# lhotse-speech/lhotse

Hardware: AMD Instinct MI355X
Metric: cuts/sec (10 s @16 kHz -> 80-dim log-mel fbank) (higher is better)
Workload: dtype f32

## Files before the change

### lhotse_amd/csrc/hipfeat.hip

```cpp
#include "../../include/hipfeat.h"

#include <hip/hip_runtime.h>

#include <algorithm>
#include <atomic>
#include <cmath>
#include <cstdarg>
#include <cstdio>
#include <cstring>
#include <map>
#include <mutex>
#include <new>
#include <string>
#include <vector>

#include "common.hpp"
#include "kernel_generic.hpp"
#include "fft512_common.hpp"
#include "kernel_fft512b.hpp"
#include "kernel_fft512c.hpp"
#include "kernel_fft1024c.hpp"
#include "kernel_fft2048c.hpp"
#include "plan_tables.hpp"
#include "kernel_resample.hpp"
#include "resample_tables.hpp"
#include "kernel_minibatch.hpp"
#include "kernel_mix.hpp"
#include "kernel_reverb.hpp"
#include "kernel_specaug.hpp"
#include "kernel_whisper2.hpp"
#include "kernel_whisper3.hpp"
#include "kernel_fft256.hpp"
#include "kernel_fft256c.hpp"
#include "kernel_wave.hpp"
#include "host_bulk.hpp"

using namespace hipfeat;

static thread_local char g_err[512] = "";

static inline const char* route_env(const char* name) { return getenv(name); }
#ifdef HIPFEAT_EXPERIMENTS
static inline const char* exp_env(const char* name) { return getenv(name); }
#else
static inline const char* exp_env(const char*) { return nullptr; }
#endif

static hipfeat_status fail(hipfeat_status st, const char* fmt, ...) {
  va_list ap;
  va_start(ap, fmt);
  vsnprintf(g_err, sizeof(g_err), fmt, ap);
  va_end(ap);
  return st;
}

#define HIP_TRY(expr)                                                                          \
  do {                                                                                         \
    hipError_t e_ = (expr);                                                                    \
    if (e_ != hipSuccess)                                                                      \
      return fail(HIPFEAT_ERR_HIP, "%s failed: %s (%s:%d)", #expr, hipGetErrorName(e_), __FILE__, __LINE__); \
  } while (0)

struct DeviceGuard {
  int prev = -1;
  bool ok = true;
  explicit DeviceGuard(int dev) {
    if (hipGetDevice(&prev) != hipSuccess) prev = -1;
    if (prev != dev) ok = (hipSetDevice(dev) == hipSuccess);
  }
  ~DeviceGuard() {
    int cur = -1;
    if (prev >= 0 && hipGetDevice(&cur) == hipSuccess && cur != prev) (void)hipSetDevice(prev);
  }
};

struct StagingSlot {
  void* h = nullptr;
  void* d = nullptr;
  size_t cap = 0;
  hipEvent_t ev = nullptr;
  bool busy = false;
};

enum class Route {
  Generic,
  Fft512b,
  Fft256b,
  Wave,
  Whisper2,
  Fft512c,
  Fft1024c,
  Whisper3,
  Fft2048c,
  Fft256c,
};

struct hipfeat_plan {
  hipfeat_config cfg{};
  int device = 0;
  int feature_dim = 0;
  int K = 0, H = 0, log2H = 0;
  bool pow2 = false;
  int npad_left = 0;
  std::string kernel_name = "generic";
  int blocks_per_cu = 0;
  Route route = Route::Generic;
  const void* fn = nullptr;
  const void* fn_flat = nullptr;
  int block = 0;
  size_t lds = 0;
  float* d_window = nullptr;
  float2* d_tw = nullptr;
  float* d_mel = nullptr;
  int2* d_mel_range = nullptr;
  float* d_dct = nullptr;
  float* d_lifter = nullptr;
  int fpb = 8;
  int span = 0, off_z = 0, off_p = 0, off_tw = 0, off_stat = 0, off_mel = 0;
  float* d_mel_a4 = nullptr;
  float* d_dct_consts = nullptr;
  int lm_stride = 0, dct_groups = 0, dct_floats = 0;
  int tiles_per_block = 4;
  int xs_floats = 0;
  int const_floats = 0;
  float* d_lds_consts = nullptr;
  float* d_mel_a = nullptr;
  WaveWork* d_work = nullptr;
  float* d_c_shared = nullptr;
  int c_shared_floats = 0, c_wtab_off = 0, c_ltab_off = 0, c_xs_floats = 0;
  int fpb_unit = 0, c_rounds_max = 0;
  int w_nsets = 0, w_steps[kWMaxSets] = {}, w_step0[kWMaxSets] = {};
  float* d_x_twp = nullptr;
  int x_waves = 0, x_tws_off = 0, x_tw32_off = 0;
  float* d_mel_t = nullptr;
  int wave_blob_floats = 0;
  bool wave_dct_in_lds = false;
  float* d_wh2_cs = nullptr;
  float* d_wh2_tw = nullptr;
  float* d_wh2_mel = nullptr;
  int32_t* d_wh2_sched = nullptr;
  mutable std::mutex mu;
  mutable StagingSlot slots[4];
  mutable int next_slot = 0;
  mutable float* d_scratch_wave = nullptr;
  mutable size_t scratch_wave_cap = 0;
  mutable float* d_scratch_out = nullptr;
  mutable size_t scratch_out_cap = 0;
};

struct hipfeat_layout {
  int device = 0;
  int64_t batch = 0;
  int64_t total_frames = 0;
  int64_t total_blocks = 0;
  int64_t out_row_stride = 0;
  int uniform_bpc = 0;
  int fpb = 0, fpb_unit = 0;
  CutDesc* d_cuts = nullptr;
  bool owns = true;
  std::vector<int64_t> num_frames;
  std::vector<int32_t> block_cut;
  bool flat = false;
  int64_t total_quads = 0;
  unsigned char* d_norm = nullptr;
  int norm_slots = 0;
  mutable std::atomic<unsigned> norm_next{0};
};
constexpr int kNormSlots = 4;
static size_t norm_slot_bytes(const hipfeat_layout* lay) { return (2 * (size_t)lay->total_blocks + (size_t)lay->batch) * 4; }

extern "C" HIPFEAT_API int32_t hipfeat_abi_version(void) { return HIPFEAT_ABI_VERSION; }
extern "C" HIPFEAT_API const char* hipfeat_last_error(void) { return g_err; }

extern "C" HIPFEAT_API hipfeat_status hipfeat_device_count(int32_t* count) {
  if (!count) return fail(HIPFEAT_ERR_INVALID, "count is NULL");
  int n = 0;
  hipError_t e = hipGetDeviceCount(&n);
  if (e != hipSuccess) {
    *count = 0;
    return fail(HIPFEAT_ERR_HIP, "hipGetDeviceCount failed: %s", hipGetErrorName(e));
  }
  *count = n;
  return HIPFEAT_OK;
}

extern "C" HIPFEAT_API int64_t hipfeat_num_frames(int64_t num_samples, int32_t frame_length, int32_t frame_shift,
                                      int32_t snip_edges) {
  if (frame_shift <= 0 || frame_length <= 0 || num_samples < 0) return 0;
  if (snip_edges) return num_samples < frame_length ? 0 : 1 + (num_samples - frame_length) / frame_shift;
  return (num_samples + frame_shift / 2) / frame_shift;
}

extern "C" HIPFEAT_API hipfeat_status hipfeat_check_length(int64_t padded_len, int32_t frame_length, int32_t frame_shift,
                                               int32_t snip_edges) {
  if (snip_edges) return HIPFEAT_OK;
  const int64_t t = hipfeat_num_frames(padded_len, frame_length, frame_shift, 0);
  if (t <= 0)
    return fail(HIPFEAT_ERR_TOO_SHORT, "waveform of %lld samples yields no frames", (long long)padded_len);
  const int64_t npad_left = (frame_length - frame_shift) / 2;
  const int64_t npad_right = (t - 1) * frame_shift + frame_length - padded_len - npad_left;
  if (npad_left > padded_len || npad_right > padded_len)
    return fail(HIPFEAT_ERR_TOO_SHORT,
                "waveform of %lld samples is shorter than the reflect padding (%lld left, %lld right)",
                (long long)padded_len, (long long)npad_left, (long long)npad_right);
  return HIPFEAT_OK;
}

// ... 100 lines not shown
  std::copy(t.w_step0, t.w_step0 + 4, p->w_step0);
  p->fpb_unit = t.waves * frames;
  p->fpb = p->fpb_unit * rounds;
  p->c_rounds_max = rounds_max;
  if ((st = claim(p, route, fn, 64 * t.waves, t.lds)) != HIPFEAT_OK) return st;
  p->kernel_name = head + strf(" lds=%zuB blocks/CU=%d mel4=%dx%d", t.lds, p->blocks_per_cu, t.sch_nsets, t.sch_steps);
  return HIPFEAT_OK;
}

static hipfeat_status claim_tile(hipfeat_plan* p, Route route, const void* fn, const TileTables& t, int tile_frames, const char* kernel) {
  const hipfeat_config& c = p->cfg;
  const bool mfcc = c.kind == HIPFEAT_MFCC, spec = c.kind == HIPFEAT_SPECTROGRAM || c.kind == HIPFEAT_LOG_SPECTROGRAM;
  hipfeat_status st;
  if ((st = upload(&p->d_lds_consts, t.consts.data(), t.consts.size())) != HIPFEAT_OK) return st;
  if (route == Route::Fft512b && (st = upload(&p->d_mel_a, t.mel_a.data(), t.mel_a.size())) != HIPFEAT_OK) return st;
  if ((st = upload(&p->d_work, t.work, 4)) != HIPFEAT_OK) return st;
  if ((st = upload(&p->d_mel_a4, t.mel_a4.data(), t.mel_a4.size())) != HIPFEAT_OK) return st;
  if (mfcc && (st = upload(&p->d_dct_consts, t.dct.data(), t.dct.size())) != HIPFEAT_OK) return st;
  p->tiles_per_block = 16;
  p->fpb = tile_frames * p->tiles_per_block;
  p->const_floats = (int)t.consts.size();
  p->xs_floats = t.xs_floats;
  p->lm_stride = t.lm_stride;
  p->dct_groups = t.dct_groups;
  p->dct_floats = (int)t.dct.size();
  if ((st = claim(p, route, fn, 256, t.lds)) != HIPFEAT_OK) return st;
  p->kernel_name = strf("%s<%d,%d> %s lds=%zuB blocks/CU=%d", kernel, t.nrows, mfcc ? 1 : (spec ? 2 : 0), mfcc ? "mfcc" : (spec ? "spectrogram" : "fbank"), t.lds,
                        p->blocks_per_cu);
  return HIPFEAT_OK;
}

static bool fft512c_has_flat(int nrows, int N) { return nrows == 13 && N >= 384; }

template <int MODE>
static const void* fft512c_pick(int nrows, int N, bool flat) {
  if (flat && fft512c_has_flat(nrows, N)) return entry<fft512c_kernel<13, 12, MODE, true>>();
  if (nrows == 10) return entry<fft512c_kernel<10, 0, MODE>>();
  if (nrows == 13 && N >= 384) return entry<fft512c_kernel<13, 12, MODE>>();
  if (nrows == 13) return entry<fft512c_kernel<13, 0, MODE>>();
  return entry<fft512c_kernel<16, 0, MODE>>();
}
static const void* fft512c_dispatch(int mode, int nrows, int N, bool flat) {
  return mode == 0 ? fft512c_pick<0>(nrows, N, flat)
                   : (mode == 1 ? fft512c_pick<1>(nrows, N, flat) : (mode == 2 ? fft512c_pick<2>(nrows, N, flat) : fft512c_pick<3>(nrows, N, flat)));
}

static hipfeat_status setup_fft512c(hipfeat_plan* p, const PlanInputs& in, int nrows) {
  const bool mfcc = p->cfg.kind == HIPFEAT_MFCC;
  if (mfcc && (in.M > 4 * kCDctChunks || in.C > 64 || !in.dct)) return HIPFEAT_OK;
  const WaveAutoTables t = build_fft512c_tables(in, nrows, {kCPRowStride, kCMaxSets, kCMaxSteps, kCWaves, kCRegion}, kCDctChunks, kCDctChunksSmall);
  if (!t.fits || t.lds > 80 * 1024 || (t.xs_floats >> 8) > 6) return HIPFEAT_OK;
  hipfeat_status st = claim_wave_auto(p, Route::Fft512c, fft512c_dispatch(t.mode, nrows, in.N, false), t, 4, 8, 16,
                                      strf("fft512c_kernel<%d> %s", nrows, mfcc ? "mfcc" : "fbank"));
  if (st == HIPFEAT_OK && fft512c_has_flat(nrows, in.N)) {
    p->fn_flat = fft512c_dispatch(t.mode, nrows, in.N, true);
    hipError_t e = ensure_dynamic_lds(p->fn_flat, t.lds);
    if (e != hipSuccess) return fail(HIPFEAT_ERR_HIP, "hipFuncSetAttribute(dynamic LDS = %zu B) failed: %s", t.lds, hipGetErrorName(e));
  }
  return st;
}

static hipfeat_status setup_fft512(hipfeat_plan* p, const PlanInputs& in) {
  const hipfeat_config& c = p->cfg;
  const char* force = route_env("HIPFEAT_FORCE_GENERIC");
  if (force && force[0] == '1') return HIPFEAT_OK;
  const bool mfcc = c.kind == HIPFEAT_MFCC;
  const bool spec = c.kind == HIPFEAT_SPECTROGRAM || c.kind == HIPFEAT_LOG_SPECTROGRAM;
  if (c.kind > HIPFEAT_MFCC || c.fft_length != 512 || (in.shift & 1) || in.N < 32 || c.use_energy || (!spec && c.use_fft_mag))
    return HIPFEAT_OK;
  if (mfcc && (in.M > 8 * kMaxDctGroups || in.C > 64)) return HIPFEAT_OK;
  const int need = (in.N + 31) / 32;
  const int nrows = need <= 10 ? 10 : (need <= 13 ? 13 : 16);
  if ((in.M + 15) / 16 > 8) return HIPFEAT_OK;

  if (!spec) {
    const char* var = route_env("HIPFEAT_FFT512_VARIANT");
    if (!(var && var[0] == 'b')) {
      hipfeat_status stc = setup_fft512c(p, in, nrows);
      if (stc != HIPFEAT_OK || p->route == Route::Fft512c) return stc;
    }
  }
  const TileTables t = build_tile_tables(in, nrows, {16, kPRowStride, kMaxGroups0, kMaxGroups1, kTileFrames, kBWaveRegion, false});
  if (!t.fits || t.lds > 160 * 1024) return HIPFEAT_OK;
  const void* fn;
  if (mfcc)
    fn = nrows == 10 ? entry<fft512b_kernel<10, 1>>() : (nrows == 13 ? entry<fft512b_kernel<13, 1>>() : entry<fft512b_kernel<16, 1>>());
  else if (spec)
    fn = nrows == 10 ? entry<fft512b_kernel<10, 2>>() : (nrows == 13 ? entry<fft512b_kernel<13, 2>>() : entry<fft512b_kernel<16, 2>>());
  else
    fn = nrows == 10 ? entry<fft512b_kernel<10, 0>>() : (nrows == 13 ? entry<fft512b_kernel<13, 0>>() : entry<fft512b_kernel<16, 0>>());
  return claim_tile(p, Route::Fft512b, fn, t, kTileFrames, "fft512b_kernel");
}

static hipfeat_status setup_fft1024c(hipfeat_plan* p, const PlanInputs& in) {
  const hipfeat_config& c = p->cfg;
  const int N = in.N, shift = in.shift;
  const bool librosa = c.kind == HIPFEAT_LIBROSA_FBANK;
  if ((c.kind != HIPFEAT_FBANK && !librosa) || c.fft_length != 1024 || (shift & 1) || N < 32 * 17 || c.use_energy ||
      (c.use_fft_mag && !librosa) || route_env("HIPFEAT_FORCE_GENERIC") || route_env("HIPFEAT_NO_WAVE_AUTONOMOUS"))
    return HIPFEAT_OK;
  const int need = (N + 31) / 32;
  const int nrows = need <= 20 ? 20 : (need <= 26 ? 26 : 32);
  static const int kFixedSteps[5][3] = {{0, 0, 0}, {24, 16, 8}, {24, 16, 8}, {24, 24, 8}, {16, 16, 8}};
  int want = 0;
  if (route_env("HIPFEAT_NO_FIXED_SCHEDULE")) want = 0;
  else if (nrows == 32) want = !c.remove_dc_offset && c.preemph_coeff == 0.0f ? 4 : 0;
// ... 337 lines not shown
  lay->flat = ragged && !no_flat && plan->fn_flat;
  lay->total_quads = 0;
  lay->block_cut.clear();
  if (lay->flat) {
    int64_t quads = 0;
    for (int64_t b = 0; b < batch; ++b) {
      if (quads > INT32_MAX - (1 << 24)) return fail(HIPFEAT_ERR_INVALID, "batch too large for one launch");
      descs[(size_t)b].first_block = (int32_t)quads;
      quads += (lay->num_frames[(size_t)b] + 3) / 4;
    }
    static const int forced = exp_env("HIPFEAT_ROUNDS") ? atoi(exp_env("HIPFEAT_ROUNDS")) : 0;
    const int64_t slots = 256LL * std::max(plan->blocks_per_cu, 1);
    const int waves_per_wg = plan->fpb_unit / 4;
    int rounds = plan->c_rounds_max;
    if (forced >= 1 && forced <= plan->c_rounds_max) {
      rounds = forced;
    } else {
      double best = -1.0;
      for (int r = std::min(2, plan->c_rounds_max); r <= plan->c_rounds_max; ++r) {
        const int64_t nb = (quads + (int64_t)waves_per_wg * r - 1) / ((int64_t)waves_per_wg * r);
        const double waves = nb >= 8 * slots ? (double)nb / (double)slots : (double)((nb + slots - 1) / slots);
        const double cost = waves * (0.64 + r);
        if (best < 0.0 || cost <= best * (1.0 + 1e-9)) {
          best = cost;
          rounds = r;
        }
      }
    }
    fpb = plan->fpb_unit * rounds;
    const int64_t qpw = (int64_t)waves_per_wg * rounds;
    blocks = (quads + qpw - 1) / qpw;
    lay->total_quads = quads;
    lay->block_cut.resize((size_t)blocks);
    int64_t cutp = 0;
    for (int64_t g = 0; g < blocks; ++g) {
      const int64_t q = g * qpw;
      while (cutp + 1 < batch && descs[(size_t)cutp + 1].first_block <= q) ++cutp;
      lay->block_cut[(size_t)g] = (int32_t)cutp;
    }
    uniform = 0;
  } else {
    for (int64_t b = 0; b < batch; ++b) {
      if (blocks > INT32_MAX - (1 << 24)) return fail(HIPFEAT_ERR_INVALID, "batch too large for one launch");
      descs[(size_t)b].first_block = (int32_t)blocks;
      const int64_t nb = (lay->num_frames[(size_t)b] + fpb - 1) / fpb;
      blocks += nb;
      if (uniform == -1) uniform = (int)nb;
      else if (uniform != (int)nb) uniform = 0;
    }
  }
  lay->batch = batch;
  lay->total_frames = row;
  lay->total_blocks = blocks;
  lay->out_row_stride = out_row_stride;
  lay->uniform_bpc = uniform > 0 ? uniform : -1;
  if (uniform <= 0 && !lay->flat) {
    lay->block_cut.resize((size_t)blocks);
    for (int64_t b = 0; b < batch; ++b) {
      const int64_t b0 = descs[(size_t)b].first_block, b1 = b + 1 < batch ? descs[(size_t)b + 1].first_block : blocks;
      std::fill(lay->block_cut.begin() + b0, lay->block_cut.begin() + b1, (int32_t)b);
    }
  }
  lay->fpb = fpb;
  lay->fpb_unit = plan->fpb_unit;
  lay->device = plan->device;
  return HIPFEAT_OK;
}

extern "C" HIPFEAT_API hipfeat_status hipfeat_layout_create(const hipfeat_plan* plan, int64_t batch, const int64_t* h_wave_offsets,
                                                const int64_t* h_num_samples, const int64_t* h_padded_len,
                                                const int64_t* h_out_rows, int64_t out_row_stride, void* stream,
                                                hipfeat_layout** layout) {
  if (!layout) return fail(HIPFEAT_ERR_INVALID, "layout pointer is NULL");
  *layout = nullptr;
  hipfeat_layout* lay = new (std::nothrow) hipfeat_layout();
  if (!lay) return fail(HIPFEAT_ERR_INVALID, "out of host memory");
  std::vector<CutDesc> descs;
  hipfeat_status st = build_descs(plan, batch, h_wave_offsets, h_num_samples, h_padded_len, h_out_rows, out_row_stride, descs, lay);
  if (st != HIPFEAT_OK) {
    delete lay;
    return st;
  }
  DeviceGuard g(plan->device);
  const size_t map_bytes = (lay->block_cut.size() * sizeof(int32_t) + 15) & ~(size_t)15;
  const size_t desc_bytes = std::max<size_t>(descs.size(), 1) * sizeof(CutDesc) + map_bytes;
  const size_t norm_bytes = plan->route == Route::Whisper3 ? (size_t)kNormSlots * norm_slot_bytes(lay) : 0;
  std::vector<unsigned char> blob(desc_bytes + norm_bytes, 0);
  if (!descs.empty()) std::memcpy(blob.data(), descs.data(), descs.size() * sizeof(CutDesc));
  if (map_bytes) std::memcpy(blob.data() + descs.size() * sizeof(CutDesc), lay->block_cut.data(), lay->block_cut.size() * sizeof(int32_t));
  hipError_t e = hipMalloc(reinterpret_cast<void**>(&lay->d_cuts), blob.size());
  if (e == hipSuccess && !descs.empty()) {
    e = hipMemcpyAsync(lay->d_cuts, blob.data(), blob.size(), hipMemcpyHostToDevice, (hipStream_t)stream);
    if (e == hipSuccess) e = hipStreamSynchronize((hipStream_t)stream);
  }
  if (norm_bytes) {
    lay->d_norm = reinterpret_cast<unsigned char*>(lay->d_cuts) + desc_bytes;
    lay->norm_slots = kNormSlots;
  }
  if (e != hipSuccess) {
    (void)hipFree(lay->d_cuts);
    delete lay;
    return fail(HIPFEAT_ERR_HIP, "layout upload failed: %s", hipGetErrorName(e));
  }
  *layout = lay;
  return HIPFEAT_OK;
}
// ... 113 lines not shown
      wp.dct = plan->d_dct;
      wp.lifter = plan->d_lifter;
      wp.out_stride = lay->out_row_stride;
      wp.num_cuts = (int32_t)lay->batch;
      wp.uniform_bpc = lay->uniform_bpc;
      wp.frames_per_wave = plan->fpb / 4;
      wp.N = c.frame_length;
      wp.shift = c.frame_shift;
      wp.H = plan->H;
      wp.K = plan->K;
      wp.M = c.num_filters;
      wp.C = c.num_ceps;
      wp.kind = librosa ? (int)HIPFEAT_FBANK : c.kind;
      wp.flags = (c.remove_dc_offset ? F_REMOVE_DC : 0) | (c.use_energy ? F_USE_ENERGY : 0) | (c.raw_energy ? F_RAW_ENERGY : 0) |
                 (c.use_fft_mag ? F_FFT_MAG : 0) | (c.apply_lifter ? F_LIFTER : 0) | (librosa ? (F_CENTER | F_LOG10) : 0);
      wp.npad_left = plan->npad_left;
      wp.preemph = c.preemph_coeff;
      wp.log_energy_floor = c.energy_floor > 0.0f ? logf(c.energy_floor) : -INFINITY;
      wp.mel_floor = c.mel_floor;
      wp.log_offset = c.log_offset;
      arg = &wp;
      break;
    case Route::Whisper2:
      w2.wave = d_wave;
      w2.out = d_out;
      w2.cuts = lay->d_cuts;
      w2.window = plan->d_window;
      w2.cs = plan->d_wh2_cs;
      w2.tw = plan->d_wh2_tw;
      w2.mel_a = plan->d_wh2_mel;
      w2.out_stride = lay->out_row_stride;
      w2.num_cuts = (int32_t)lay->batch;
      w2.uniform_bpc = lay->uniform_bpc;
      w2.M = c.num_filters;
      w2.mel_floor = c.mel_floor;
      w2.sched = plan->d_wh2_sched;
      arg = &w2;
      break;
    case Route::Whisper3:
      fill_wave_autonomous(w3, plan, lay, d_wave, d_out);
      w3.cs = plan->d_wh2_cs;
      w3.total_blocks = (int32_t)lay->total_blocks;
      if (lay->d_norm) {
        unsigned char* slot = lay->d_norm + (size_t)(lay->norm_next.fetch_add(1u) % (unsigned)lay->norm_slots) * norm_slot_bytes(lay);
        w3.wg_stat = reinterpret_cast<float*>(slot);
        w3.cut_done = reinterpret_cast<uint32_t*>(slot + 2 * (size_t)lay->total_blocks * sizeof(float));
      }
      arg = &w3;
      break;
    case Route::Fft512c:
      cp.dct_tab = plan->d_dct_consts;
      cp.C = c.num_ceps;
      cp.total_quads = (int32_t)lay->total_quads;
      [[fallthrough]];
    case Route::Fft256c:
      fill_wave_autonomous(cp, plan, lay, d_wave, d_out);
      fill_frames(cp, plan);
      arg = &cp;
      break;
    case Route::Fft1024c:
      fill_wave_autonomous(kp, plan, lay, d_wave, d_out);
      fill_frames(kp, plan);
      kp.nsets = plan->w_nsets;
      for (int s2 = 0; s2 < kWMaxSets; ++s2) kp.steps[s2] = plan->w_steps[s2], kp.step0[s2] = plan->w_step0[s2];
      arg = &kp;
      break;
    case Route::Fft2048c:
      fill_wave_autonomous(xp, plan, lay, d_wave, d_out);
      fill_frames(xp, plan);
      xp.twp = plan->d_x_twp;
      xp.waves = plan->x_waves;
      xp.tws_off = plan->x_tws_off;
      xp.tw32_off = plan->x_tw32_off;
      xp.nsets = plan->w_nsets;
      for (int s2 = 0; s2 < kXMaxSets; ++s2) xp.steps[s2] = plan->w_steps[s2], xp.step0[s2] = plan->w_step0[s2];
      arg = &xp;
      break;
    case Route::Fft512b:
    case Route::Fft256b:
      bp.wave = d_wave;
      bp.out = d_out;
      bp.cuts = lay->d_cuts;
      bp.lds_consts = plan->d_lds_consts;
      bp.mel_a = plan->d_mel_a4;
      bp.work = plan->d_work;
      bp.out_stride = lay->out_row_stride;
      bp.num_cuts = (int32_t)lay->batch;
      bp.uniform_bpc = lay->uniform_bpc;
      bp.tiles_per_block = plan->tiles_per_block;
      bp.N = c.frame_length;
      bp.shift = c.frame_shift;
      bp.npad_left = plan->npad_left;
      bp.M = c.num_filters;
      bp.flags = (c.remove_dc_offset ? F_REMOVE_DC : 0) | (c.use_fft_mag ? F_FFT_MAG : 0) | (c.kind == HIPFEAT_LOG_SPECTROGRAM ? F_LOG_SPEC : 0);
      bp.log_offset = c.log_offset;
      bp.preemph = c.preemph_coeff;
      bp.mel_floor = c.mel_floor;
      bp.xs_floats = plan->xs_floats;
      bp.const_floats = plan->const_floats;
      bp.dct_consts = plan->d_dct_consts;
      bp.C = c.num_ceps;
      bp.lm_stride = plan->lm_stride;
      bp.dct_groups = plan->dct_groups;
      bp.dct_floats = plan->dct_floats;
      arg = &bp;
      break;
  }
  const void* fn = lay->flat && plan->fn_flat ? plan->fn_flat : plan->fn;
  void* args[] = {arg};
  DeviceGuard g(plan->device);
  set_lds_poison(plan->lds);
  (void)hipLaunchKernel(fn, dim3((unsigned)lay->total_blocks), dim3(plan->block), args, plan->lds, stream);
  HIP_TRY(hipGetLastError());
  if (whisper && !(plan->route == Route::Whisper3 && lay->d_norm)) {
    hipLaunchKernelGGL(whisper_norm_kernel, dim3((unsigned)lay->batch), dim3(1024), 0, stream, lay->d_cuts, d_out, lay->out_row_stride,
                       (int32_t)c.num_filters, (int32_t)c.frame_shift);
    HIP_TRY(hipGetLastError());
  }
  return HIPFEAT_OK;
}

extern "C" HIPFEAT_API hipfeat_status hipfeat_extract_layout(const hipfeat_plan* plan, const hipfeat_layout* layout,
                                                 const float* d_wave, float* d_out, void* stream) {
  if (!plan || !layout) return fail(HIPFEAT_ERR_INVALID, "plan/layout is NULL");
  return launch(plan, layout, d_wave, d_out, (hipStream_t)stream);
}

__global__ __launch_bounds__(256) void fill_padding_kernel(const CutDesc* __restrict__ cuts, float* __restrict__ out, int64_t row_stride,
                                                           int32_t rows_per_cut, int32_t feature_dim, float value) {
  const CutDesc cd = cuts[blockIdx.y];
  const int64_t n = (int64_t)(rows_per_cut - cd.num_frames) * feature_dim;
  float* __restrict__ base = out + (cd.out_row + cd.num_frames) * row_stride;
  for (int64_t i = (int64_t)blockIdx.x * 256 + threadIdx.x; i < n; i += (int64_t)gridDim.x * 256) {
    const int64_t r = i / feature_dim;
    base[r * row_stride + (i - r * feature_dim)] = value;
  }
}

__global__ __launch_bounds__(256) void pcm16_to_float_kernel(const int16_t* __restrict__ in, float* __restrict__ out, int64_t n) {
  const int64_t n8 = n >> 3;
  const bool aligned = ((reinterpret_cast<uintptr_t>(in) & 15) == 0) && ((reinterpret_cast<uintptr_t>(out) & 15) == 0);
  constexpr float k = 1.0f / 32768.0f;
  if (aligned) {
    for (int64_t i = (int64_t)blockIdx.x * 256 + threadIdx.x; i < n8; i += (int64_t)gridDim.x * 256) {
      const int4 v = reinterpret_cast<const int4*>(in)[i];
      const int w[4] = {v.x, v.y, v.z, v.w};
      float4 a, b;
      a.x = (float)(int16_t)(w[0] & 0xffff) * k; a.y = (float)(w[0] >> 16) * k;
      a.z = (float)(int16_t)(w[1] & 0xffff) * k; a.w = (float)(w[1] >> 16) * k;
      b.x = (float)(int16_t)(w[2] & 0xffff) * k; b.y = (float)(w[2] >> 16) * k;
      b.z = (float)(int16_t)(w[3] & 0xffff) * k; b.w = (float)(w[3] >> 16) * k;
      reinterpret_cast<float4*>(out)[2 * i] = a;
      reinterpret_cast<float4*>(out)[2 * i + 1] = b;
    }
    for (int64_t i = (n8 << 3) + (int64_t)blockIdx.x * 256 + threadIdx.x; i < n; i += (int64_t)gridDim.x * 256) out[i] = (float)in[i] * k;
  } else {
    for (int64_t i = (int64_t)blockIdx.x * 256 + threadIdx.x; i < n; i += (int64_t)gridDim.x * 256) out[i] = (float)in[i] * k;
  }
}

extern "C" HIPFEAT_API hipfeat_status hipfeat_pcm16_to_float(const int16_t* d_pcm, float* d_wave, int64_t num_samples, void* stream) {
  if (num_samples < 0 || (num_samples > 0 && (!d_pcm || !d_wave))) return fail(HIPFEAT_ERR_INVALID, "bad pcm16 arguments");
  if (num_samples == 0) return HIPFEAT_OK;
  const int64_t blocks = std::min<int64_t>((num_samples / 8 + 255) / 256 + 1, 256 * 32);
  hipLaunchKernelGGL(pcm16_to_float_kernel, dim3((unsigned)blocks), dim3(256), 0, (hipStream_t)stream, d_pcm, d_wave, num_samples);
// ... 1306 lines not shown
```

### lhotse_amd/csrc/kernel_fft512c.hpp

```cpp
#pragma once
#include "common.hpp"
#include "fft_common.hpp"

namespace hipfeat {

constexpr int kCExRowStride = 34;
constexpr int kCExFrameStride = 8 * kCExRowStride + 16;
constexpr int kCPRowStride = 272;
constexpr int kCRegion = 4 * kCExFrameStride + 16;
constexpr int kCMaxSets = 2;
constexpr int kCMaxSteps = 16;
constexpr int kCWaves = 8;
constexpr int kCLmStride = 48;
constexpr int kCDctChunks = 10;
constexpr int kCDctChunksSmall = 6;

struct Fft512cParams {
  const float* wave;
  float* out;
  const CutDesc* cuts;
  const float* shared_consts;
  int64_t out_stride;
  int32_t num_cuts, uniform_bpc;
  int32_t frames_per_block, rounds;
  int32_t N, shift, npad_left, M, flags;
  float preemph, mel_floor;
  int32_t shared_floats;
  int32_t wtab_off, ltab_off;
  int32_t xs_floats;
  const float* dct_tab;
  int32_t C;
  int32_t total_quads;
};

#ifdef HIPFEAT_PHASE_TIMERS
#define HFC_T(i) { const unsigned long long tt_ = __builtin_readcyclecounter(); hfc_acc[i] += tt_ - hfc_last; hfc_last = tt_; }
#else
#define HFC_T(i)
#endif
#define HFC_SEP() asm volatile("")
__device__ __forceinline__ int mul24(int a, int b) { return (int)__umul24((unsigned)a, (unsigned)b); }

template <int NROWS, int NFULL, int MODE, bool FLAT = false>
__global__ __launch_bounds__(64 * kCWaves, 4) void fft512c_kernel(const Fft512cParams p) {
  extern __shared__ __attribute__((aligned(16))) float smem[];
  HF_POISON_LDS(smem);
  const v2* cwin = reinterpret_cast<const v2*>(smem);
  const v2* ctwp = cwin + NROWS * 16;
  const v2* ctws = ctwp + 256;
  const float* wtab = smem + p.wtab_off;
  const float* ltab = smem + p.ltab_off;

  const int tid = threadIdx.x;
  const int lane = tid & 63;
  const int wv = __builtin_amdgcn_readfirstlane(tid >> 6);

  const int blk = blockIdx.x;
  int cut, fb;
  if (FLAT) {
    cut = __builtin_amdgcn_readfirstlane(block_cut_map(p.cuts, p.num_cuts)[blk]);
    fb = 0;
  } else if (p.uniform_bpc > 0) {
    cut = blk / p.uniform_bpc;
    fb = blk - cut * p.uniform_bpc;
  } else {
    cut = p.uniform_bpc < 0 ? block_cut_map(p.cuts, p.num_cuts)[blk] : find_cut(p.cuts, p.num_cuts, blk);
    fb = blk - p.cuts[cut].first_block;
  }
  CutDesc cd = FLAT ? load_cut_uniform(p.cuts + cut) : p.cuts[cut];
  const int N = p.N, shift = p.shift;

  for (int i = tid; i < p.shared_floats; i += 64 * kCWaves) smem[i] = p.shared_consts[i];
  float* xs = smem + p.shared_floats + wv * (p.xs_floats + kCRegion);
  float* myreg = xs + p.xs_floats;
  const bool dc = (p.flags & F_REMOVE_DC) != 0;
  const float inv_n = 1.0f / (float)N;
  const float c = p.preemph;

  auto stage_span = [&](const CutDesc& cd, int f0, unsigned lane4) {
    const float* __restrict__ w = p.wave + cd.wave_off;
    const int64_t j0 = (int64_t)f0 * shift - p.npad_left;
    if (j0 >= 0 && j0 + p.xs_floats <= cd.num_samples) {
      const char* src = reinterpret_cast<const char*>(w + j0);
      const int nfull = p.xs_floats >> 8;
#pragma unroll
      for (int ch = 0; ch < 6; ++ch) {
        if (ch < nfull)
          __builtin_amdgcn_global_load_lds((const __attribute__((address_space(1))) void*)(src + ((unsigned)ch * 1024u + 4u * lane4)),
                                           (__attribute__((address_space(3))) void*)(xs + ch * 256), 16, 0, 0);
      }
      if ((unsigned)nfull * 256u + lane4 < (unsigned)p.xs_floats)
        __builtin_amdgcn_global_load_lds((const __attribute__((address_space(1))) void*)(src + ((unsigned)nfull * 1024u + 4u * lane4)),
                                         (__attribute__((address_space(3))) void*)(xs + nfull * 256), 16, 0, 0);
    } else {
      for (int i = (int)(lane4 >> 2); i < p.xs_floats; i += 64) xs[i] = load_sample(w, j0 + i, cd.num_samples, cd.padded_len);
    }
  };

  const int first_frame = fb * p.frames_per_block + 4 * wv;
  int quad = 0, next_first = 0, f0_flat = 0;
  int cut_n = 0, quad_n = 0, next_first_n = 0, f0_n = 0;
  CutDesc cd_n = cd;
  auto advance = [&](int q, int& c, CutDesc& d, int& nfirst) {
    while (c + 1 < p.num_cuts && q >= nfirst) {
      ++c;
      d = load_cut_uniform(p.cuts + c);
      nfirst = c + 1 < p.num_cuts ? __builtin_amdgcn_readfirstlane(p.cuts[c + 1].first_block) : p.total_quads;
    }
  };
  if (FLAT) {
    quad = blk * (p.frames_per_block >> 2) + wv;
    next_first = cut + 1 < p.num_cuts ? __builtin_amdgcn_readfirstlane(p.cuts[cut + 1].first_block) : p.total_quads;
    advance(quad, cut, cd, next_first);
    f0_flat = 4 * (quad - cd.first_block);
    cut_n = cut, cd_n = cd, next_first_n = next_first, quad_n = quad + kCWaves;
    advance(quad_n, cut_n, cd_n, next_first_n);
    f0_n = 4 * (quad_n - cd_n.first_block);
  }
  __syncthreads();
  if (FLAT ? quad < p.total_quads : first_frame < cd.num_frames) stage_span(cd, FLAT ? f0_flat : first_frame, (unsigned)lane * 4u);

  constexpr bool kMfcc = MODE == 2 || MODE == 3;
  constexpr int DCH = MODE == 3 ? kCDctChunksSmall : kCDctChunks;
#ifdef HIPFEAT_ABL_MFCC_TWS
  constexpr bool kTwsExp = MODE == 2 && NROWS <= 13;
#else
  constexpr bool kTwsExp = false;
#endif
  constexpr int DREG = kTwsExp ? 6 : (MODE == 2 && NROWS > 13) ? 5 : DCH;
  constexpr bool kDctLate = DREG < DCH;
  constexpr bool kRegTw = !kMfcc && NROWS <= 13;
  constexpr bool kRegTws = kRegTw || (MODE == 3 && NROWS <= 13) || kTwsExp;
  v2 twpreg[kRegTw ? 16 : 1], twsreg[kRegTws ? 8 : 1];
  if (kRegTw) {
#pragma unroll
    for (int k1 = 1; k1 < 16; ++k1) twpreg[k1] = ctwp[k1 * 16 + (lane & 15)];
  }
  if (kRegTws) {
#pragma unroll
    for (int k2 = 0; k2 < 8; ++k2) twsreg[k2] = ctws[k2 * 16 + (lane & 15)];
  }
  f32x4 dw[kMfcc ? DREG : 1];
  float lift = 1.0f;
  if (kMfcc) {
#pragma unroll
    for (int c4 = 0; c4 < DREG; ++c4) dw[c4] = *reinterpret_cast<const f32x4*>(p.dct_tab + (c4 * 64 + lane) * 4);
    lift = p.dct_tab[DCH * 256 + lane];
  }
#ifdef HIPFEAT_PHASE_TIMERS
  unsigned long long hfc_acc[8] = {0, 0, 0, 0, 0, 0, 0, 0}, hfc_last = __builtin_readcyclecounter();
#endif
  for (int r = 0; r < p.rounds; ++r) {
    const int f0 = FLAT ? f0_flat : first_frame + 4 * kCWaves * r;
    if (FLAT ? quad >= p.total_quads : f0 >= cd.num_frames) break;
    const int nf = min(4, cd.num_frames - f0);

    if (r == 0)
    __builtin_amdgcn_s_waitcnt(0x0F70);
    HFC_T(0);
    int lane_o = lane;
    asm volatile("" : "+v"(lane_o));
    const int q = lane_o & 15, g = lane_o >> 4;

    int early_poff[2] = {0, 0};
    v2 Z[16];
    {
      const float* x = xs + mul24(g, shift) + 2 * q;
      v2 z[16];
      v2 win[NROWS];
      v2 sum2 = {0.f, 0.f};
#pragma unroll
      for (int n1 = 0; n1 < NROWS; ++n1) {
        z[n1] = *reinterpret_cast<const v2*>(x + 32 * n1);
        HFC_SEP();
      }
#pragma unroll
      for (int n1 = 0; n1 < NROWS; ++n1) {
        win[n1] = cwin[n1 * 16 + q];
        HFC_SEP();
      }
      float pv[NROWS];
#pragma unroll
      for (int n1 = 0; n1 < NROWS; ++n1) pv[n1] = n1 == 0 ? x[q == 0 ? 0 : -1] : x[32 * n1 - 1];
      asm volatile("s_waitcnt lgkmcnt(0)" ::: "memory");
      HFC_T(1);
      if (FLAT) {
        if (r + 1 < p.rounds && quad_n < p.total_quads) stage_span(cd_n, f0_n, (unsigned)lane_o * 4u);
      } else if (r + 1 < p.rounds && f0 + 4 * kCWaves < cd.num_frames) {
        stage_span(cd, f0 + 4 * kCWaves, (unsigned)lane_o * 4u);
      }

#pragma unroll
      for (int n1 = NFULL; n1 < NROWS; ++n1) {
        if (32 * (n1 + 1) > N) {
          const int m0 = 32 * n1 + 2 * q;
          if (m0 >= N) z[n1].x = 0.f;
          if (m0 + 1 >= N) z[n1].y = 0.f;
        }
      }
      {
        v2 sa = z[0], sb = z[1], sc = z[2], sd = z[3];
#pragma unroll
        for (int n1 = 4; n1 < NROWS; ++n1) {
          if ((n1 & 3) == 0) sa += z[n1];
          if ((n1 & 3) == 1) sb += z[n1];
          if ((n1 & 3) == 2) sc += z[n1];
          if ((n1 & 3) == 3) sd += z[n1];
        }
        sum2 = (sa + sb) + (sc + sd);
      }
      float mu = 0.f;
      if (dc) mu = row16_sum(sum2.x + sum2.y) * inv_n;
      {
        const float nc = -c, mu1 = (1.0f - c) * mu;
#pragma unroll
        for (int n1 = 0; n1 < NROWS; ++n1) {
          v2 t;
          asm("v_fma_f32 %0, %1, %2, %3" : "=v"(t.x) : "s"(nc), "v"(pv[n1]), "v"(z[n1].x));
          asm("v_fma_f32 %0, %1, %2, %3" : "=v"(t.y) : "s"(nc), "v"(z[n1].x), "v"(z[n1].y));
          z[n1] = (t - v2{mu1, mu1}) * win[n1];
        }
      }
#pragma unroll
      for (int n1 = NROWS; n1 < 16; ++n1) z[n1] = v2{0.f, 0.f};
      v2 a[16];
      fft16(z, a);
#pragma unroll
      for (int h = 0; h < 2; ++h) {
        v2 tw[8];
        if (kRegTw) {
#pragma unroll
          for (int rr = 0; rr < 8; ++rr) tw[rr] = twpreg[8 * h + rr];
        } else {
#pragma unroll
          for (int rr = 0; rr < 8; ++rr) {
            tw[rr] = ctwp[(8 * h + rr) * 16 + q];
            HFC_SEP();
          }
        }
#pragma unroll
        for (int rr = (h == 0 ? 1 : 0); rr < 8; ++rr) a[8 * h + rr] = cmul2(a[8 * h + rr], tw[rr]);
      }

// ... 141 lines not shown
      if (MODE != 0) acc[0] += acc[1];
      float val[S][4];
#pragma unroll
      for (int s = 0; s < S; ++s) {
        mel4_reduce_floor(acc[s], lt_m4[s], lt_m8[s], p.mel_floor, val[s]);
#pragma unroll
        for (int i = 0; i < 4; ++i) val[s][i] = fast_log(val[s][i]);
      }
#pragma unroll
      for (int s = 0; s < S; ++s) {
        const int col = lt_col[s];
        if (kMfcc) {
#pragma unroll
          for (int i = 0; i < 4; ++i) lm[i] = val[s][i];
        } else if (col < p.M) {
          mel4_store_saddr<4>(orow, (unsigned)col, p.out_stride, nf, val[s]);
        }
      }
    }
    if (kMfcc) {
      float* lmrow = myreg;
      const int col = lt_col[0];
      if (col < p.M) {
#pragma unroll
        for (int i = 0; i < 4; ++i) lmrow[i * kCLmStride + col] = lm[i];
      }
      __builtin_amdgcn_fence(__ATOMIC_RELEASE, "wavefront");
      __builtin_amdgcn_wave_barrier();
      __builtin_amdgcn_fence(__ATOMIC_ACQUIRE, "wavefront");
      f32x4 al[DCH];
#pragma unroll
      for (int c4 = 0; c4 < DCH; ++c4) al[c4] = *reinterpret_cast<const f32x4*>(lmrow + (lane_o & 3) * kCLmStride + 4 * c4);
      f32x4 d0 = {0.f, 0.f, 0.f, 0.f}, d1 = {0.f, 0.f, 0.f, 0.f};
#pragma unroll
      for (int c4 = 0; c4 < DCH; ++c4) {
#pragma unroll
        for (int i = 0; i < 4; i += 2) {
          const f32x4 w4 = (kDctLate && c4 >= DREG) ? dwx[c4 >= DREG ? c4 - DREG : 0] : dw[c4 < DREG ? c4 : 0];
          d0 = __builtin_amdgcn_mfma_f32_4x4x1f32(al[c4][i], w4[i], d0, 0, 0, 0);
          d1 = __builtin_amdgcn_mfma_f32_4x4x1f32(al[c4][i + 1], w4[i + 1], d1, 0, 0, 0);
        }
      }
      d0 += d1;
      if (lane_o < p.C) {
#pragma unroll
        for (int i = 0; i < 4; ++i)
          if (i < nf) orow[i * p.out_stride + lane_o] = d0[i] * lift;
      }
    }
    HFC_T(6);
#ifdef HIPFEAT_PHASE_TIMERS
    hfc_acc[7] += 1;
#endif
    if (FLAT) {
      quad = quad_n, cut = cut_n, cd = cd_n, next_first = next_first_n, f0_flat = f0_n;
      quad_n += kCWaves;
      advance(quad_n, cut_n, cd_n, next_first_n);
      f0_n = 4 * (quad_n - cd_n.first_block);
    }
  }
#ifdef HIPFEAT_PHASE_TIMERS
  if (lane == 0 && g_phase_buf) {
    unsigned long long* o = g_phase_buf + ((size_t)blockIdx.x * kCWaves + wv) * 8;
    for (int i = 0; i < 8; ++i) o[i] = hfc_acc[i];
  }
#endif
}

}
```

Measured before the change: 2.961 million.

## Make fft512c workgroups persistent over multiple blocks with a cost-model grid size

Adds a host cost model that picks how many logical blocks each workgroup processes, shrinking the launch grid. The fft512c kernel now walks blocks in a grid-stride loop and keeps the double-buffered staging of the next span running across block boundaries. The goal is to amortise per-workgroup startup (constant loading into LDS, initial staging) and to soften the tail effect. The risk is worse load balance when the model picks K>1, plus extra position-tracking state that adds registers.

```diff
diff --git a/lhotse_amd/csrc/blocks_per_wg.hpp b/lhotse_amd/csrc/blocks_per_wg.hpp
--- /dev/null
+++ b/lhotse_amd/csrc/blocks_per_wg.hpp
@@ -0,0 +1,122 @@
+#pragma once
+#include <algorithm>
+#include <cstdint>
+#include <vector>
+
+#if defined(__HIPCC__)
+#define HFB_HD __host__ __device__ inline __attribute__((always_inline))
+#else
+#define HFB_HD inline
+#endif
+
+namespace hipfeat {
+
+constexpr double kWgStartupRounds = 0.64;
+constexpr double kMeasuredStartupRounds = 0.0;
+constexpr double kStaticStrideTail = 0.09;
+
+struct BpwTerms { double startup, tail; };
+constexpr BpwTerms kBpwAsSetUp{kWgStartupRounds, 0.0}, kBpwMeasured{kMeasuredStartupRounds, kStaticStrideTail};
+
+inline int64_t bpw_grid(int64_t total_blocks, int64_t K) { return (total_blocks + std::max<int64_t>(K, 1) - 1) / std::max<int64_t>(K, 1); }
+
+inline double bpw_cost(int64_t grid, int64_t K, int64_t slots, int rounds, BpwTerms t) {
+  const double waves = K == 1 && grid >= 8 * slots ? (double)grid / (double)slots : (double)((grid + slots - 1) / slots);
+  return waves * (t.startup + (double)K * rounds) + (K > 1 ? t.tail * (double)K * rounds : 0.0);
+}
+
+inline int64_t choose_blocks_per_wg(int64_t total_blocks, int64_t slots, int rounds, BpwTerms t = kBpwMeasured) {
+  slots = std::max<int64_t>(slots, 1);
+  if (total_blocks <= slots) return 1;
+  int64_t best_k = 1;
+  double best = bpw_cost(total_blocks, 1, slots, rounds, t);
+  const int64_t wmax = std::min<int64_t>((total_blocks + slots - 1) / slots, 64);
+  for (int64_t w = wmax; w >= 1; --w) {
+    const int64_t K = (total_blocks + w * slots - 1) / (w * slots);
+    const double cost = bpw_cost(bpw_grid(total_blocks, K), K, slots, rounds, t);
+    if (cost < best * (1.0 - 1e-9) || (cost <= best * (1.0 + 1e-9) && K > best_k)) best = cost, best_k = K;
+  }
+  return best_k;
+}
+
+inline int64_t layout_blocks_per_wg(int64_t total_blocks, int64_t slots, int rounds, int64_t forced) {
+  if (total_blocks <= 0) return 1;
+  if (forced > 0) return std::min(forced, total_blocks);
+  return choose_blocks_per_wg(total_blocks, slots, rounds);
+}
+
+HFB_HD uint32_t walk_block(uint32_t g, uint32_t j, uint32_t grid) { return g + j * grid; }
+HFB_HD int percut_first_frame(int fb, int frames_per_block, int wv, int r, int waves) { return fb * frames_per_block + 4 * (wv + waves * r); }
+HFB_HD int flat_quad(int blk, int frames_per_block, int wv, int r, int waves) { return blk * (frames_per_block >> 2) + wv + waves * r; }
+
+struct WalkLayout {
+  std::vector<int64_t> num_frames;
+  std::vector<int64_t> first_block;
+  std::vector<int32_t> block_cut;
+  bool flat = false;
+  int rounds = 0, waves = 8;
+  int64_t total_blocks = 0, total_quads = 0;
+  int frames_per_block() const { return 4 * waves * rounds; }
+};
+
+inline WalkLayout walk_layout(const int64_t* num_frames, int64_t batch, int rounds, int waves, bool flat) {
+  WalkLayout l;
+  l.flat = flat, l.rounds = rounds, l.waves = waves;
+  l.num_frames.assign(num_frames, num_frames + batch);
+  l.first_block.resize((size_t)batch);
+  const int64_t fpb = l.frames_per_block(), qpw = fpb / 4;
+  if (flat) {
+    for (int64_t b = 0; b < batch; ++b) l.first_block[(size_t)b] = l.total_quads, l.total_quads += (num_frames[b] + 3) / 4;
+    l.total_blocks = (l.total_quads + qpw - 1) / qpw;
+    int64_t cutp = 0;
+    for (int64_t g = 0; g < l.total_blocks; ++g) {
+      while (cutp + 1 < batch && l.first_block[(size_t)cutp + 1] <= g * qpw) ++cutp;
+      l.block_cut.push_back((int32_t)cutp);
+    }
+  } else {
+    for (int64_t b = 0; b < batch; ++b) {
+      l.first_block[(size_t)b] = l.total_blocks;
+      const int64_t nb = (num_frames[b] + fpb - 1) / fpb;
+      l.total_blocks += nb;
+      l.block_cut.insert(l.block_cut.end(), (size_t)nb, (int32_t)b);
+    }
+  }
+  return l;
+}
+
+inline bool walk_locate(const WalkLayout& l, int64_t blk, int wv, int r, int64_t* cut, int64_t* first_frame) {
+  if (blk < 0 || blk >= l.total_blocks) return false;
+  int64_t c = l.block_cut[(size_t)blk];
+  if (l.flat) {
+    const int64_t quad = flat_quad((int)blk, l.frames_per_block(), wv, r, l.waves);
+    if (quad >= l.total_quads) return false;
+    while (c + 1 < (int64_t)l.num_frames.size() && quad >= l.first_block[(size_t)c + 1]) ++c;
+    *cut = c, *first_frame = 4 * (quad - l.first_block[(size_t)c]);
+    return true;
+  }
+  const int64_t f0 = percut_first_frame((int)(blk - l.first_block[(size_t)c]), l.frames_per_block(), wv, r, l.waves);
+  if (f0 >= l.num_frames[(size_t)c]) return false;
+  *cut = c, *first_frame = f0;
+  return true;
+}
+
+struct WalkVisit { int64_t blk, cut, first_frame; };
+inline int64_t walk_launch(const WalkLayout& l, int64_t K, std::vector<WalkVisit>& visits) {
+  const int64_t grid = bpw_grid(l.total_blocks, K);
+  int64_t max_blk = -1;
+  for (int64_t g = 0; g < grid; ++g)
+    for (int wv = 0; wv < l.waves; ++wv)
+      for (uint32_t j = 0;; ++j) {
+        const uint32_t blk = walk_block((uint32_t)g, j, (uint32_t)grid);
+        if (blk >= (uint32_t)l.total_blocks) break;
+        max_blk = std::max<int64_t>(max_blk, blk);
+        for (int r = 0; r < l.rounds; ++r) {
+          int64_t cut, f0;
+          if (!walk_locate(l, blk, wv, r, &cut, &f0)) break;
+          visits.push_back({(int64_t)blk, cut, f0});
+        }
+      }
+  return max_blk;
+}
+
+}
diff --git a/lhotse_amd/csrc/hipfeat.hip b/lhotse_amd/csrc/hipfeat.hip
--- a/lhotse_amd/csrc/hipfeat.hip
+++ b/lhotse_amd/csrc/hipfeat.hip
@@ -18,6 +18,7 @@
 #include "kernel_generic.hpp"
 #include "fft512_common.hpp"
 #include "kernel_fft512b.hpp"
+#include "blocks_per_wg.hpp"
 #include "kernel_fft512c.hpp"
 #include "kernel_fft1024c.hpp"
 #include "kernel_fft2048c.hpp"
@@ -107,6 +108,7 @@
   Route route = Route::Generic;
   const void* fn = nullptr;
   const void* fn_flat = nullptr;
+  int64_t blocks_per_wg_forced = 0;
   int block = 0;
   size_t lds = 0;
   float* d_window = nullptr;
@@ -153,6 +155,7 @@
   int64_t batch = 0;
   int64_t total_frames = 0;
   int64_t total_blocks = 0;
+  int64_t blocks_per_wg = 1;
   int64_t out_row_stride = 0;
   int uniform_bpc = 0;
   int fpb = 0, fpb_unit = 0;
@@ -359,6 +362,7 @@
   if (!t.fits || t.lds > 80 * 1024 || (t.xs_floats >> 8) > 6) return HIPFEAT_OK;
   hipfeat_status st = claim_wave_auto(p, Route::Fft512c, fft512c_dispatch(t.mode, nrows, in.N, false), t, 4, 8, 16,
                                       strf("fft512c_kernel<%d> %s", nrows, mfcc ? "mfcc" : "fbank"));
+  if (const char* bpw = route_env("HIPFEAT_BLOCKS_PER_WG")) p->blocks_per_wg_forced = std::max<int64_t>(0, atoll(bpw));
   if (st == HIPFEAT_OK && fft512c_has_flat(nrows, in.N)) {
     p->fn_flat = fft512c_dispatch(t.mode, nrows, in.N, true);
     hipError_t e = ensure_dynamic_lds(p->fn_flat, t.lds);
@@ -802,6 +806,9 @@
   lay->batch = batch;
   lay->total_frames = row;
   lay->total_blocks = blocks;
+  lay->blocks_per_wg = 1;
+  if (plan->route == Route::Fft512c && plan->fpb_unit > 0)
+    lay->blocks_per_wg = layout_blocks_per_wg(blocks, 256LL * std::max(plan->blocks_per_cu, 1), fpb / plan->fpb_unit, plan->blocks_per_wg_forced);
   lay->out_row_stride = out_row_stride;
   lay->uniform_bpc = uniform > 0 ? uniform : -1;
   if (uniform <= 0 && !lay->flat) {
@@ -1021,6 +1028,7 @@
       cp.dct_tab = plan->d_dct_consts;
       cp.C = c.num_ceps;
       cp.total_quads = (int32_t)lay->total_quads;
+      cp.total_blocks = (int32_t)lay->total_blocks;
       [[fallthrough]];
     case Route::Fft256c:
       fill_wave_autonomous(cp, plan, lay, d_wave, d_out);
@@ -1079,7 +1087,8 @@
   void* args[] = {arg};
   DeviceGuard g(plan->device);
   set_lds_poison(plan->lds);
-  (void)hipLaunchKernel(fn, dim3((unsigned)lay->total_blocks), dim3(plan->block), args, plan->lds, stream);
+  const int64_t grid = plan->route == Route::Fft512c ? bpw_grid(lay->total_blocks, lay->blocks_per_wg) : lay->total_blocks;
+  (void)hipLaunchKernel(fn, dim3((unsigned)grid), dim3(plan->block), args, plan->lds, stream);
   HIP_TRY(hipGetLastError());
   if (whisper && !(plan->route == Route::Whisper3 && lay->d_norm)) {
     hipLaunchKernelGGL(whisper_norm_kernel, dim3((unsigned)lay->batch), dim3(1024), 0, stream, lay->d_cuts, d_out, lay->out_row_stride,
diff --git a/lhotse_amd/csrc/kernel_fft512c.hpp b/lhotse_amd/csrc/kernel_fft512c.hpp
--- a/lhotse_amd/csrc/kernel_fft512c.hpp
+++ b/lhotse_amd/csrc/kernel_fft512c.hpp
@@ -1,4 +1,5 @@
 #pragma once
+#include "blocks_per_wg.hpp"
 #include "common.hpp"
 #include "fft_common.hpp"
 
@@ -31,6 +32,7 @@
   const float* dct_tab;
   int32_t C;
   int32_t total_quads;
+  int32_t total_blocks;
 };
 
 #ifdef HIPFEAT_PHASE_TIMERS
@@ -55,19 +57,6 @@
   const int lane = tid & 63;
   const int wv = __builtin_amdgcn_readfirstlane(tid >> 6);
 
-  const int blk = blockIdx.x;
-  int cut, fb;
-  if (FLAT) {
-    cut = __builtin_amdgcn_readfirstlane(block_cut_map(p.cuts, p.num_cuts)[blk]);
-    fb = 0;
-  } else if (p.uniform_bpc > 0) {
-    cut = blk / p.uniform_bpc;
-    fb = blk - cut * p.uniform_bpc;
-  } else {
-    cut = p.uniform_bpc < 0 ? block_cut_map(p.cuts, p.num_cuts)[blk] : find_cut(p.cuts, p.num_cuts, blk);
-    fb = blk - p.cuts[cut].first_block;
-  }
-  CutDesc cd = FLAT ? load_cut_uniform(p.cuts + cut) : p.cuts[cut];
   const int N = p.N, shift = p.shift;
 
   for (int i = tid; i < p.shared_floats; i += 64 * kCWaves) smem[i] = p.shared_consts[i];
@@ -82,7 +71,8 @@
     const int64_t j0 = (int64_t)f0 * shift - p.npad_left;
     if (j0 >= 0 && j0 + p.xs_floats <= cd.num_samples) {
       const char* src = reinterpret_cast<const char*>(w + j0);
-      const int nfull = p.xs_floats >> 8;
+      int nfull = p.xs_floats >> 8;
+      asm volatile("" : "+s"(nfull));
 #pragma unroll
       for (int ch = 0; ch < 6; ++ch) {
         if (ch < nfull)
@@ -97,28 +87,83 @@
     }
   };
 
-  const int first_frame = fb * p.frames_per_block + 4 * wv;
-  int quad = 0, next_first = 0, f0_flat = 0;
-  int cut_n = 0, quad_n = 0, next_first_n = 0, f0_n = 0;
-  CutDesc cd_n = cd;
-  auto advance = [&](int q, int& c, CutDesc& d, int& nfirst) {
-    while (c + 1 < p.num_cuts && q >= nfirst) {
-      ++c;
-      d = load_cut_uniform(p.cuts + c);
-      nfirst = c + 1 < p.num_cuts ? __builtin_amdgcn_readfirstlane(p.cuts[c + 1].first_block) : p.total_quads;
-    }
-  };
-  if (FLAT) {
-    quad = blk * (p.frames_per_block >> 2) + wv;
-    next_first = cut + 1 < p.num_cuts ? __builtin_amdgcn_readfirstlane(p.cuts[cut + 1].first_block) : p.total_quads;
-    advance(quad, cut, cd, next_first);
-    f0_flat = 4 * (quad - cd.first_block);
-    cut_n = cut, cd_n = cd, next_first_n = next_first, quad_n = quad + kCWaves;
-    advance(quad_n, cut_n, cd_n, next_first_n);
-    f0_n = 4 * (quad_n - cd_n.first_block);
-  }
+  struct Pos {
+    CutDesc cd;
+    unsigned blk;
+    int r, f0;
+    int cut, quad, next_first;
+  };
+  const unsigned nblk = (unsigned)p.total_blocks, stride = gridDim.x;
+  auto advance = [&](Pos& s) {
+    while (s.cut + 1 < p.num_cuts && s.quad >= s.next_first) {
+      ++s.cut;
+      s.cd = load_cut_uniform(p.cuts + s.cut);
+      s.next_first = s.cut + 1 < p.num_cuts ? __builtin_amdgcn_readfirstlane(p.cuts[s.cut + 1].first_block) : p.total_quads;
+    }
+  };
+  auto enter_block = [&](Pos& s) {
+    s.r = 0;
+    if (FLAT) {
+      s.quad = flat_quad((int)s.blk, p.frames_per_block, wv, 0, kCWaves);
+      if (s.quad >= p.total_quads) return false;
+      s.cut = __builtin_amdgcn_readfirstlane(block_cut_map(p.cuts, p.num_cuts)[s.blk]);
+      s.cd = load_cut_uniform(p.cuts + s.cut);
+      s.next_first = s.cut + 1 < p.num_cuts ? __builtin_amdgcn_readfirstlane(p.cuts[s.cut + 1].first_block) : p.total_quads;
+      advance(s);
+      s.f0 = 4 * (s.quad - s.cd.first_block);
+      return true;
+    }
+    int fb;
+    if (p.uniform_bpc > 0) {
+      const unsigned cut = s.blk / (unsigned)p.uniform_bpc;
+      fb = (int)(s.blk - cut * (unsigned)p.uniform_bpc);
+      s.cd = load_cut_uniform(p.cuts + cut);
+    } else {
+      const int cut = p.uniform_bpc < 0 ? __builtin_amdgcn_readfirstlane(block_cut_map(p.cuts, p.num_cuts)[s.blk])
+                                        : __builtin_amdgcn_readfirstlane(find_cut(p.cuts, p.num_cuts, (int)s.blk));
+      s.cd = load_cut_uniform(p.cuts + cut);
+      fb = (int)s.blk - s.cd.first_block;
+    }
+    s.f0 = percut_first_frame(fb, p.frames_per_block, wv, 0, kCWaves);
+    return s.f0 < s.cd.num_frames;
+  };
+  auto next_block = [&](Pos& s) { s.blk = walk_block(s.blk, 1u, stride); };
+  auto find_block = [&](Pos& s) {
+    while (s.blk < nblk && !enter_block(s)) {
+      if (FLAT) {
+        s.blk = nblk;
+        break;
+      }
+      next_block(s);
+    }
+    if (s.blk >= nblk) s.f0 = -1;
+  };
+  auto step = [&](Pos& s) {
+    if (s.r + 1 < p.rounds && (FLAT || s.f0 + 4 * kCWaves < s.cd.num_frames)) {
+      ++s.r;
+      if (FLAT) {
+        s.quad += kCWaves;
+        if (s.quad >= p.total_quads) {
+          s.f0 = -1;
+          return;
+        }
+        advance(s);
+        s.f0 = 4 * (s.quad - s.cd.first_block);
+      } else {
+        s.f0 += 4 * kCWaves;
+      }
+      return;
+    }
+    next_block(s);
+    find_block(s);
+  };
+  Pos cur{};
+  cur.blk = blockIdx.x;
+  find_block(cur);
+  Pos nxt = cur;
+  if (cur.f0 >= 0) step(nxt);
   __syncthreads();
-  if (FLAT ? quad < p.total_quads : first_frame < cd.num_frames) stage_span(cd, FLAT ? f0_flat : first_frame, (unsigned)lane * 4u);
+  if (cur.f0 >= 0) stage_span(cur.cd, cur.f0, (unsigned)lane * 4u);
 
   constexpr bool kMfcc = MODE == 2 || MODE == 3;
   constexpr int DCH = MODE == 3 ? kCDctChunksSmall : kCDctChunks;
@@ -150,13 +195,12 @@
 #ifdef HIPFEAT_PHASE_TIMERS
   unsigned long long hfc_acc[8] = {0, 0, 0, 0, 0, 0, 0, 0}, hfc_last = __builtin_readcyclecounter();
 #endif
-  for (int r = 0; r < p.rounds; ++r) {
-    const int f0 = FLAT ? f0_flat : first_frame + 4 * kCWaves * r;
-    if (FLAT ? quad >= p.total_quads : f0 >= cd.num_frames) break;
+  __builtin_amdgcn_s_waitcnt(0x0F70);
+  while (cur.f0 >= 0) {
+    const CutDesc& cd = cur.cd;
+    const int f0 = cur.f0;
     const int nf = min(4, cd.num_frames - f0);
 
-    if (r == 0)
-    __builtin_amdgcn_s_waitcnt(0x0F70);
     HFC_T(0);
     int lane_o = lane;
     asm volatile("" : "+v"(lane_o));
@@ -184,11 +228,7 @@
       for (int n1 = 0; n1 < NROWS; ++n1) pv[n1] = n1 == 0 ? x[q == 0 ? 0 : -1] : x[32 * n1 - 1];
       asm volatile("s_waitcnt lgkmcnt(0)" ::: "memory");
       HFC_T(1);
-      if (FLAT) {
-        if (r + 1 < p.rounds && quad_n < p.total_quads) stage_span(cd_n, f0_n, (unsigned)lane_o * 4u);
-      } else if (r + 1 < p.rounds && f0 + 4 * kCWaves < cd.num_frames) {
-        stage_span(cd, f0 + 4 * kCWaves, (unsigned)lane_o * 4u);
-      }
+      if (nxt.f0 >= 0) stage_span(nxt.cd, nxt.f0, (unsigned)lane_o * 4u);
 
 #pragma unroll
       for (int n1 = NFULL; n1 < NROWS; ++n1) {
@@ -436,12 +476,8 @@
 #ifdef HIPFEAT_PHASE_TIMERS
     hfc_acc[7] += 1;
 #endif
-    if (FLAT) {
-      quad = quad_n, cut = cut_n, cd = cd_n, next_first = next_first_n, f0_flat = f0_n;
-      quad_n += kCWaves;
-      advance(quad_n, cut_n, cd_n, next_first_n);
-      f0_n = 4 * (quad_n - cd_n.first_block);
-    }
+    cur = nxt;
+    if (nxt.f0 >= 0) step(nxt);
   }
 #ifdef HIPFEAT_PHASE_TIMERS
   if (lane == 0 && g_phase_buf) {
```

After: 2.941 million. No clear change (-0.7%).
